# kfkq/DQMC

Hardware: AMD Instinct MI355X
Metric: MC sweeps/sec, 2D Hubbard N=256 Ltau=200 (higher is better)
Workload: dtype f64; 1 GPU; cfg3: 16x16 Hubbard U=8.0 beta=8.0 Ltau=200 n_stab=10 t=1 mu=-0.1; chains_per_gpu=1, n_chains_total=1, parallelism=independent chains, 1 gpu x 1 chain

## Files before the change

dqmc_amd/abi.py:

```python
from __future__ import annotations

import ctypes as C
import os
from typing import Optional, Tuple

import numpy as np

c_double_p = C.POINTER(C.c_double)
c_int64_p = C.POINTER(C.c_int64)
c_int32_p = C.POINTER(C.c_int32)
c_uint8_p = C.POINTER(C.c_uint8)
c_uint32_p = C.POINTER(C.c_uint32)
c_uint64_p = C.POINTER(C.c_uint64)


class Stats(C.Structure):
    _fields_ = [("acc_rate", C.c_double), ("max_err", C.c_double), ("sum_err", C.c_double),
                ("n_err", C.c_double), ("n_accepted", C.c_int64), ("n_proposed", C.c_int64)]

    @property
    def mean_err(self) -> float:
        return self.sum_err / self.n_err if self.n_err else 0.0


class DqmcError(RuntimeError):
    def __init__(self, code: int, msg: str):
        super().__init__(f"[{code}] {msg}")
        self.code = code


ABI_SYMBOLS = [
    "last_error", "backend", "device_count",
    "to_ldr", "ldr_mul_mat", "mat_mul_ldr", "ldr_mul_ldr", "inv_I_plus_ldr", "inv_I_plus_ldr_mul_ldr",
    "gemm", "rank1_update",
    "create", "create_batch", "n_chains", "destroy", "set_fields", "get_fields", "init", "get_G", "set_G", "get_logdet",
    "n_stack", "get_stack", "sweep_0_to_beta", "sweep_beta_to_0", "sync", "get_stats",
    "wrap_forward", "wrap_backward", "local_update_slice", "calculate_Bbar", "global_action", "set_checkerboard",
    "update_kernel_time", "set_profiling", "slice_path", "debug_snapshot", "debug_gt_check",
    "measure_equal_time", "measure_accumulate", "measure_fetch",
    "sweep_unequal_time", "get_G_tau", "half_warp", "measure_unequal_time", "measure_unequal_fetch",
    "comm_unique_id", "comm_create_rccl", "comm_create_callbacks", "comm_destroy", "comm_rank", "comm_world_size",
    "comm_transport", "comm_barrier", "comm_allreduce_sum", "comm_selftest", "partner_rank", "replica_exchange_round",
    "replica_exchange_batch",
    "rng_seed", "rng_state", "rng_draw", "rng_fill_time",
]

UNIQUE_ID_BYTES = 128
SENDRECV_FN = C.CFUNCTYPE(C.c_int, C.c_void_p, C.c_void_p, C.c_void_p, C.c_size_t, C.c_int, C.c_int)


class ExchangeResult(C.Structure):
    _fields_ = [("partner", C.c_int), ("decider", C.c_int), ("accepted", C.c_int), ("pad", C.c_int),
                ("S", C.c_double), ("S_prime", C.c_double), ("S_partner", C.c_double), ("S_prime_partner", C.c_double),
# ... 47 lines not shown
        if self.has_symbol("slice_path"):
            g("slice_path").argtypes = [C.c_void_p]
        if self.has_symbol("measure_equal_time"):
            g("measure_equal_time").argtypes = [C.c_void_p, C.c_int, C.c_int, c_double_p, c_double_p]
            g("measure_accumulate").argtypes = [C.c_void_p, C.c_int, C.c_int]
            g("measure_fetch").argtypes = [C.c_void_p, c_double_p, c_double_p, c_int64_p, C.c_int]
        if self.has_symbol("sweep_unequal_time"):
            g("sweep_unequal_time").argtypes = [C.c_void_p]
            g("get_G_tau").argtypes = [C.c_void_p, C.c_int, C.c_int, c_double_p]
            g("measure_unequal_time").argtypes = [C.c_void_p, C.c_int, C.c_int, C.c_int, c_double_p]
            g("measure_unequal_fetch").argtypes = [C.c_void_p, c_double_p, c_int64_p, C.c_int]
        if self.has_symbol("half_warp"):
            g("half_warp").argtypes = [C.c_void_p, c_double_p, c_double_p, C.c_int, C.c_int, c_double_p]
        if self.has_symbol("debug_snapshot"):
            g("debug_snapshot").argtypes = [C.c_void_p, c_double_p, C.c_void_p, C.c_void_p, C.c_void_p]
        if self.has_symbol("debug_gt_check"):
            g("debug_gt_check").argtypes = [C.c_void_p, C.c_int, c_double_p, c_int64_p]
        if self.has_symbol("replica_exchange_round"):
            g("comm_unique_id").argtypes = [C.c_void_p]
            g("comm_create_rccl").argtypes = [C.POINTER(C.c_void_p), C.c_void_p, C.c_int, C.c_int, C.c_int]
            g("comm_create_callbacks").argtypes = [C.POINTER(C.c_void_p), C.c_int, C.c_int, SENDRECV_FN, C.c_void_p]
            g("comm_destroy").argtypes = [C.c_void_p]; g("comm_destroy").restype = None
            g("comm_rank").argtypes = [C.c_void_p]; g("comm_world_size").argtypes = [C.c_void_p]
            g("comm_transport").argtypes = [C.c_void_p]; g("comm_transport").restype = C.c_char_p
            g("comm_barrier").argtypes = [C.c_void_p]; g("comm_selftest").argtypes = [C.c_void_p]
            g("comm_allreduce_sum").argtypes = [C.c_void_p, c_double_p, C.c_int]
            g("partner_rank").argtypes = [C.c_int, C.c_int, C.c_int]
            g("replica_exchange_round").argtypes = [C.c_void_p, C.c_void_p, C.c_int, C.c_double, C.POINTER(ExchangeResult)]
        if self.has_symbol("replica_exchange_batch"):
            g("replica_exchange_batch").argtypes = [C.c_void_p, C.c_void_p, C.c_int, c_double_p, C.POINTER(ExchangeResult)]
# ... 354 lines not shown
        out = np.empty(self.C * 3 * (self.nt + 1) * L1 * L2); cnt = np.zeros(1, dtype=np.int64)
        self._c("measure_unequal_fetch", _p(out), cnt.ctypes.data_as(c_int64_p), 1 if reset else 0)
        return self._ut_cube(out, L1, L2), int(cnt[0])

    def debug_snapshot(self):
        ns = self.n_stack()
        we = np.zeros(ns); acc = np.zeros(self.nt, np.int32); sw = np.zeros(80, np.uint32); ep = C.c_uint(0)
        self._c("debug_snapshot", _p(we), acc.ctypes.data, sw.ctypes.data, C.byref(ep))
        return dict(wrap_err=we, accepted=acc, sync_words=sw, slice_epoch=int(ep.value))

    def debug_gt_check(self, on: bool):
        err = np.zeros(self.C); cnt = np.zeros(1, dtype=np.int64)
        self._c("debug_gt_check", int(bool(on)), _p(err), cnt.ctypes.data_as(c_int64_p))
        return err, int(cnt[0])

    def slice_path(self) -> int:
        return int(self.lib._sym("slice_path")(self._h))

    def set_profiling(self, on: bool):
        self._c("set_profiling", int(bool(on)))

    def update_kernel_time(self):
        ms = C.c_double(0.0); nl = C.c_int64(0); na = C.c_int64(0)
        self._c("update_kernel_time", C.cast(C.byref(ms), c_double_p), C.cast(C.byref(nl), c_int64_p), C.cast(C.byref(na), c_int64_p))
        return ms.value, nl.value, na.value
```

dqmc_amd/csrc/common.h:

```cpp
#pragma once

#include <hip/hip_runtime.h>
#include <cstdint>
#include <memory>
#include <string>

struct dqmc_engine;

namespace dq {

constexpr int WAVE = 64;

void set_error(const std::string& msg);
const char* get_error();

#define DQ_HIP(call)                                                                    \
    do {                                                                                \
        hipError_t _e = (call);                                                         \
        if (_e != hipSuccess) {                                                         \
            ::dq::set_error(std::string(#call) + ": " + hipGetErrorString(_e));         \
            return -2;                                              \
        }                                                                               \
    } while (0)

// ... 88 lines not shown

int launch_tri_solve(CMat R, const int* perm, long perm_stride, Mat X, CVec dg, double* scratch, long scratch_stride, int n, int n_chains, hipStream_t s);

bool gj_fused_fits(int n);
bool gj_fused_default(int n);
int launch_gj_solve(Mat A, Mat B, Mat X, Mat SA, double* tinv, int* perm, long perm_stride, int* rowpos, int* rowpos_alt, long rowpos_stride,
                    double* logabsdet, int accumulate_logdet, int* info, int n, int n_chains, bool fused, hipStream_t s);

struct UpdateTables {
    double rb[4][3];
    double delta[4][3];
    double ev[4];
    double iev[4];
    double pad[32];
};
struct UpdateDesc {
    Mat G;
    int8_t* fields; long f_stride;
    double* expv; double* invexpv; long v_stride;
    const UpdateTables* tabs;
    const int32_t* perm; const uint8_t* kprop; const double* u; long rs_stride;
    double* Upanel; double* Wpanel; long panel_stride;
    double* Cpanel = nullptr;
    int* state; long state_stride;
    double* prep; long prep_stride;
    Mat GT{nullptr, 0};
    int gt_valid = 0;
    void* slice_sync = nullptr;
    unsigned slice_epoch = 0;
    int slice_absent_tile = -1;
    int slice_absent_l = -1;
    int slice_late_tile = -1, slice_late_us = 0;
    int* info = nullptr;
    int* acc_out; long acc_stride;
    int n, nt;
};
constexpr int UPDATE_KD = 32;

struct SliceSync {
    unsigned long long seq; unsigned int error; unsigned int solo_count; unsigned int pad[12];
    unsigned int arrive[496];
};
constexpr size_t SLICE_SYNC_BYTES = 2048;
static_assert(sizeof(SliceSync) == SLICE_SYNC_BYTES, "SliceSync layout");
constexpr unsigned SLICE_EPOCH_LIMIT = 1u << 24;
constexpr unsigned SLICE_SOLO_BIT = 1u << 30, SLICE_FINAL_BIT = 1u << 31;
__host__ __device__ inline unsigned slice_tag(unsigned epoch, unsigned window) { return (epoch << 8) | window; }
enum class SlicePath { PersistentWalk, PersistentSubmatrix, Solo, Pairs, PairsTailSolo };
int launch_update_slice(SlicePath path, const UpdateDesc& d, int l, int acc_slot, int n_chains, hipStream_t s);
int launch_update_slice_sm(const UpdateDesc& d, int l, int acc_slot, int n_chains, hipStream_t s);
// ... 32 lines not shown
```

dqmc_amd/csrc/engine.hip:

```cpp
#include "common.h"
#include "../../include/dqmc_hip.h"

#include <cmath>
#include <cstdlib>
#include <cstring>
#include <map>
#include <memory>
#include <mutex>
#include <vector>

namespace dq {

static thread_local std::string g_err;
void set_error(const std::string& msg) { g_err = msg; }
const char* get_error() { return g_err.c_str(); }

int init_device_kernels(int device) {
    static std::mutex mu; static bool done[64] = {};
    std::lock_guard<std::mutex> lk(mu);
    if (device < 0 || device >= 64) { set_error("device ordinal out of range"); return -1; }
    if (done[device]) return 0;
    DQ_HIP(hipSetDevice(device));
    DQ_TRY(update_init_device()); DQ_TRY(update_sm_init_device()); DQ_TRY(qr_init_device()); DQ_TRY(qr_colown_init_device());
    done[device] = true;
    return 0;
}

struct Switches { bool qr_panel; int qr_panel_fused, gj_fused; bool qr_streaming, walk_submatrix, lu_classic, slice_multikernel; };
static const Switches& switches() {
    static const Switches sw = [] {
        const char* panel = getenv("DQMC_QR_PANEL");
        const char* fused = getenv("DQMC_QR_PANEL_FUSED");
        const char* gj = getenv("DQMC_GJ_FUSED");
        return Switches{!(panel && atoi(panel) == 0), fused ? (atoi(fused) != 0 ? 1 : 0) : -1, gj ? (atoi(gj) != 0 ? 1 : 0) : -1, getenv("DQMC_QR_STREAMING") != nullptr, getenv("DQMC_WALK_SUBMATRIX") != nullptr,
                        getenv("DQMC_LU_CLASSIC") != nullptr, getenv("DQMC_SLICE_MULTIKERNEL") != nullptr};
    }();
    return sw;
}

constexpr int GJ_MAX_N = 1024, GJ_MAX_CHAINS = 8;
constexpr int TRI_MAX_N = 640;

static QrFamily pick_qr(int n, int chains, bool allow_panel) {
    const Switches& sw = switches();
    if (sw.qr_streaming) return QrFamily::Streaming;
    if (allow_panel && sw.qr_panel && n >= 64 && n <= 1024 && n % 16 == 0 && chains <= 8) return QrFamily::Panel;
    if (n <= 256) return QrFamily::ColumnOwner;
    return qrcp_coop_workgroups(n, chains) <= 200 ? QrFamily::Cooperative : QrFamily::Streaming;
}

// ... 229 lines not shown
    Ctx ctx;
    hipStream_t s = nullptr;

    DevPtr<double> expK, invexpK;
    bool cb = false; int cb_groups = 0;
    DevPtr<int> cb_partner;
    DevPtr<double> cb_par;
    DevPtr<int8_t> fields;
    DevPtr<double> expv, invexpv;
    DevPtr<UpdateTables> tabs; DevPtr<double> tab8;
    bool gt_valid = false;
    bool gt_check = false; long long gt_checks = 0; DevPtr<double> gt_err;
    DevPtr<double> G, Gtmp, GT;
    DevPtr<double> pg_eye, pg_ones;
    DevPtr<double> bb0, bb1;
    LdrStore stack;
    LdrStore spare;
    DevPtr<double> logdet;
    DevPtr<int32_t> rs_perm; DevPtr<uint8_t> rs_k; DevPtr<double> rs_u;
    PinnedPtr h_stage;
    bool rng_seeded = false; uint64_t rng_seed = 0; uint32_t rng_first_chain = 0, rng_counter = 0;
    hipEvent_t stage_free = nullptr;
    DevPtr<double> Upanel, Wpanel;
    DevPtr<double> Cpanel;
    struct InitBatch { DevPtr<double> bb, tau; LdrStore f; } ib;
    DevPtr<int> state;
    DevPtr<double> prep;
    DevPtr<double> meas_now, meas_sum;
    struct UnequalTime { DevPtr<double> G[3], tmp, err, meas_now, meas_sum; LdrStore bt; } ut;
    bool ut_valid = false; long long ut_meas_count = 0;
// ... 181 lines not shown
        stack_valid = true;
        gt_valid = false;
        return ctx.inv_I_plus_ldr(stack.at(0), mG(), logdet.get());
    }
    int wrap_forward(int l) {
        if (cb) {
            DQ_TRY(cb_apply(mG(), Mat{nullptr, 0}, ctx.T(0), false, false, CVec(), CVec(), CVec(), CVec(), C, 4));
            gt_valid = use_gt();
            return cb_apply(ctx.T(0), Mat{GT.get(), nn}, mG(), false, true, CVec(), CVec(), iev(l), ev(l), C, 4);
        }
        DQ_TRY(ctx.gemm(CMat(expK.get(), nn), mG(), ctx.T(0)));
        gt_valid = use_gt();
        return ctx.gemm(ctx.T(0), CMat(invexpK.get(), nn), mG(), ev(l), CVec(), iev(l), 0, 0, use_gt() ? Mat{GT.get(), nn} : Mat{nullptr, 0});
    }
    bool piggyback() const { return C == 1 && !cb && n <= 256 && pg_eye != nullptr; }
    int wrap_forward_piggy(int l, const double* Pprev, double* Pnext) {
        GemmDesc g; g.A = CMat(expK.get(), 0); g.B = CMat(G.get(), (long)(Pprev - G.get())); g.C = Mat{ctx.T(0).p, (long)(Pnext - ctx.T(0).p)};
        g.rs = CVec(pg_ones.get(), (long)((expv.get() + (long)(l - 1) * n) - pg_ones.get())); g.n = n;
        DQ_TRY(launch_gemm(g, 2, s));
        gt_valid = use_gt();
        return ctx.gemm(ctx.T(0), CMat(invexpK.get(), nn), mG(), ev(l), CVec(), iev(l), 0, 0, use_gt() ? Mat{GT.get(), nn} : Mat{nullptr, 0});
    }
    int wrap_backward_piggy(int l, const double* Pprev, double* Pnext) {
        DQ_TRY(ctx.gemm(CMat(invexpK.get(), nn), mG(), ctx.T(0), CVec(), iev(l)));
        gt_valid = use_gt();
        GemmDesc g; g.A = CMat(ctx.T(0).p, (long)(Pprev - ctx.T(0).p)); g.B = CMat(expK.get(), 0); g.C = Mat{G.get(), (long)(Pnext - G.get())};
        g.ks = CVec(expv.get() + (long)l * n, 0); g.n = n;
        if (use_gt()) g.CT = Mat{GT.get(), (long)(ctx.T(1).p - GT.get())};
        return launch_gemm(g, 2, s);
    }
// ... 2 lines not shown
            DQ_TRY(cb_apply(mG(), Mat{nullptr, 0}, ctx.T(0), true, true, iev(l), ev(l), CVec(), CVec(), C, 4));
            gt_valid = use_gt();
            return cb_apply(ctx.T(0), Mat{GT.get(), nn}, mG(), true, false, CVec(), CVec(), CVec(), CVec(), C, 4);
        }
        DQ_TRY(ctx.gemm(CMat(invexpK.get(), nn), mG(), ctx.T(0), CVec(), iev(l)));
        gt_valid = use_gt();
        return ctx.gemm(ctx.T(0), CMat(expK.get(), nn), mG(), CVec(), ev(l), CVec(), 0, 0, use_gt() ? Mat{GT.get(), nn} : Mat{nullptr, 0});
    }
    bool use_gt() const { return n <= 256 || slice_path == SlicePath::PersistentSubmatrix; }
    UpdateDesc udesc() const {
        UpdateDesc d; d.G = mG(); d.fields = fields.get(); d.f_stride = (long)nt * n; d.expv = expv.get(); d.invexpv = invexpv.get(); d.v_stride = (long)nt * n;
        d.tabs = tabs.get(); d.perm = rs_perm.get(); d.kprop = rs_k.get(); d.u = rs_u.get(); d.rs_stride = (long)nt * n; d.Upanel = Upanel.get(); d.Wpanel = Wpanel.get(); d.Cpanel = Cpanel.get();
        d.panel_stride = (long)UPDATE_KD * n; d.state = state.get(); d.state_stride = 4; d.prep = prep.get(); d.prep_stride = 4L * n; d.slice_sync = is_persistent(slice_path) ? slice_sync.get() : nullptr; d.slice_epoch = slice_epoch; d.slice_absent_tile = slice_absent_tile; d.slice_absent_l = slice_absent_l; d.slice_late_tile = slice_late_tile; d.slice_late_us = slice_late_us; d.GT = Mat{GT.get(), nn}; d.gt_valid = gt_valid ? 1 : 0; d.info = ctx.info(); d.acc_out = acc.get(); d.acc_stride = nt; d.n = n; d.nt = nt;
        return d;
    }
    int local_update(int l) {
        hipEvent_t e0 = nullptr, e1 = nullptr;
        if (profiling) {
            if (ev_used == ev_pairs.size()) { hipEvent_t a, b; DQ_HIP(hipEventCreate(&a)); DQ_HIP(hipEventCreate(&b)); ev_pairs.emplace_back(a, b); }
            e0 = ev_pairs[ev_used].first; e1 = ev_pairs[ev_used].second; ++ev_used;
            DQ_HIP(hipEventRecord(e0, s));
        }
        if (is_persistent(slice_path)) {
            if (++slice_epoch >= SLICE_EPOCH_LIMIT) { DQ_HIP(hipMemsetAsync(slice_sync.get(), 0, (size_t)C * SLICE_SYNC_BYTES, s)); slice_epoch = 1; }
        }
        DQ_TRY(launch_update_slice(slice_path, udesc(), l, l, C, s));
        if (profiling) DQ_HIP(hipEventRecord(e1, s));
        return 0;
    }
    int check_stream(const char* who, const int32_t* perm, const uint8_t* kprop, const double* u, size_t rows) {
        if (!perm || !kprop || !u) { set_error(std::string(who) + ": null random-stream pointer"); return DQMC_EINVAL; }
        seen.assign((size_t)n, 0);
        for (size_t row = 0; row < rows; ++row) {
            const int32_t* pr = perm + row * n; const uint8_t* kr = kprop + row * n; const unsigned char mark = (unsigned char)(1 + (row & 1));
            if ((row & 1) == 0) std::fill(seen.begin(), seen.end(), 0);
            for (int idx = 0; idx < n; ++idx) {
                const int32_t i = pr[idx];
                if (i < 0 || i >= n || seen[i] == mark || kr[idx] > 2) { set_error(std::string(who) + ": perm is not a permutation of the sites, or kprop > 2"); return DQMC_EINVAL; }
                seen[i] = mark;
            }
        }
// ... 17 lines not shown
    int fill_stream(uint32_t h) {
        return launch_rng_fill(rs_perm.get(), rs_k.get(), rs_u.get(), n, nt, rng_seed, rng_first_chain, h, C, s);
    }
    int stage_stream(const char* who, const int32_t* perm, const uint8_t* kprop, const double* u) {
        if (perm && kprop && u) return upload_stream(perm, kprop, u);
        if (perm || kprop || u) { set_error(std::string(who) + ": pass all three random-stream arrays or none"); return DQMC_EINVAL; }
        if (!rng_seeded) { set_error(std::string(who) + ": null random-stream pointer (the engine draws its own stream only after dqmc_rng_seed)"); return DQMC_EINVAL; }
        if (rng_counter == UINT32_MAX) { set_error(std::string(who) + ": the half-sweep counter of this seed is used up (2^32 - 1)"); return DQMC_ERANGE; }
        DQ_TRY(fill_stream(rng_counter));
        ++rng_counter;
        return 0;
    }
    int sweep_fwd() {
        int n_err = 0;
        DQ_HIP(hipMemsetAsync(err.get(), 0, sizeof(double) * C * n_stack, s));
        const bool pg = piggyback();
        double* Pcur = bb0.get(); double* Pnxt = bb1.get();
        for (int l = 0; l < nt; ++l) {
            const int is = stack_idx(l), loc = local_l(l);
            if (pg && loc >= 1) { DQ_TRY(wrap_forward_piggy(l, loc == 1 ? pg_eye.get() : Pcur, Pnxt)); std::swap(Pcur, Pnxt); }
            else DQ_TRY(wrap_forward(l));
            DQ_TRY(local_update(l));
            if (loc == loc_l_end[is]) {
                std::swap(G, Gtmp);
                Mat bb;
                if (pg) {
                    if (loc == 0) DQ_TRY(launch_scale_rows(CMat(expK.get(), nn), ev(l), Mat{Pnxt, nn}, n, C, s));
                    else DQ_TRY(ctx.gemm(CMat(expK.get(), nn), CMat(Pcur, nn), Mat{Pnxt, nn}, ev(l)));
                    std::swap(Pcur, Pnxt); bb = Mat{Pcur, nn};
                } else DQ_TRY(Bbar(is, &bb));
                if (is == 0) DQ_TRY(ctx.to_ldr(bb, stack.at(0)));
                else DQ_TRY(ctx.mat_mul_ldr(bb, stack.at(is - 1), stack.at(is)));
                gt_valid = false;
                if (l == nt - 1) DQ_TRY(ctx.inv_I_plus_ldr(stack.at(is), mG(), logdet.get()));
                else DQ_TRY(ctx.inv_I_plus_ldr_mul_ldr(stack.at(is), stack.at(is + 1), mG()));
                DQ_TRY(launch_max_abs_diff(CMat(Gtmp.get(), nn), mG(), err.get() + n_err, n_stack, n, C, s));
                ++n_err;
            }
        }
        return launch_fold_stats(dstats.get(), acc.get(), nt, nt, err.get(), n_stack, n_err, n, nt, C, s);
    }
    int sweep_bwd() {
        int n_err = 0;
        DQ_HIP(hipMemsetAsync(err.get(), 0, sizeof(double) * C * n_stack, s));
        const bool pg = piggyback();
        double* Pcur = bb0.get(); double* Pnxt = bb1.get();
        for (int l = nt - 1; l >= 0; --l) {
            DQ_TRY(local_update(l));
            const int is = stack_idx(l);
            if (pg) { DQ_TRY(wrap_backward_piggy(l, local_l(l) == loc_l_end[is] ? pg_eye.get() : Pcur, Pnxt)); std::swap(Pcur, Pnxt); }
            else DQ_TRY(wrap_backward(l));
            if (local_l(l) == 0) {
                std::swap(G, Gtmp);
                Mat bb;
                if (pg) bb = Mat{Pcur, nn}; else DQ_TRY(Bbar(is, &bb));
                if (is == n_stack - 1) DQ_TRY(ctx.to_ldr(bb, stack.at(is)));
                else DQ_TRY(ctx.ldr_mul_mat(stack.at(is + 1), bb, stack.at(is)));
                gt_valid = false;
                if (l == 0) DQ_TRY(ctx.inv_I_plus_ldr(stack.at(is), mG(), logdet.get()));
                else {
                    DQ_TRY(ctx.inv_I_plus_ldr_mul_ldr(stack.at(is - 1), stack.at(is), mG(), use_gt() ? Mat{GT.get(), nn} : Mat{nullptr, 0}));
                    gt_valid = use_gt();
                    if (gt_check && gt_valid) {
                        DQ_TRY(launch_transpose_scale(mG(), ctx.T(0), CVec(), n, C, s));
                        DQ_TRY(launch_max_abs_diff(CMat(GT.get(), nn), ctx.T(0), gt_err.get(), 1, n, C, s));
                        ++gt_checks;
// ... 502 lines not shown
    DQ_HIP(hipMemcpy(st.data(), e.dstats.get(), sizeof(DevStats) * e.C, hipMemcpyDeviceToHost));
    long long acc = 0; for (auto& x : st) acc += x.n_accepted;
    if (ms) *ms = e.upd_ms; if (n_launches) *n_launches = e.upd_launches; if (n_accepted) *n_accepted = acc - e.upd_accept_base;
    e.upd_ms = 0.0; e.upd_launches = 0; e.upd_accept_base = acc;
    return 0;
}
int dqmc_debug_snapshot(dqmc_engine* h, double* wrap_err, int* accepted, unsigned int* sync_words, unsigned int* slice_epoch) {
    ENGINE_CALL(h);
    DQ_HIP(hipStreamSynchronize(e.s));
    if (wrap_err) DQ_HIP(hipMemcpy(wrap_err, e.err.get(), sizeof(double) * e.n_stack, hipMemcpyDeviceToHost));
    if (accepted) DQ_HIP(hipMemcpy(accepted, e.acc.get(), sizeof(int) * e.nt, hipMemcpyDeviceToHost));
    if (sync_words) DQ_HIP(hipMemcpy(sync_words, e.slice_sync.get(), sizeof(unsigned int) * 80, hipMemcpyDeviceToHost));
    if (slice_epoch) *slice_epoch = e.slice_epoch;
    return 0;
}
int dqmc_debug_gt_check(dqmc_engine* h, int on, double* max_err, int64_t* n_checks) {
    ENGINE_CALL(h); DQ_TRY(e.sync_and_check());
    if (!e.gt_err) { DQ_TRY(dev_alloc(e.gt_err, e.C)); DQ_HIP(hipMemset(e.gt_err.get(), 0, sizeof(double) * e.C)); }
    if (max_err) DQ_HIP(hipMemcpy(max_err, e.gt_err.get(), sizeof(double) * e.C, hipMemcpyDeviceToHost));
    if (n_checks) *n_checks = e.gt_checks;
    DQ_HIP(hipMemset(e.gt_err.get(), 0, sizeof(double) * e.C));
    e.gt_checks = 0; e.gt_check = on != 0;
    return 0;
}
int dqmc_slice_path(dqmc_engine* h) {
    if (!h) return -1;
    Engine& e = h->e;
    if (!is_persistent(e.slice_path)) return 0;
    unsigned solo = 0;
    for (int c = 0; c < e.C && !solo; ++c) {
// ... 12 lines not shown
```

dqmc_amd/csrc/gemm.hip:

```cpp
#include "common.h"
#include <cstdlib>

namespace dq {

using d4 = __attribute__((ext_vector_type(4))) double;

template <bool TRANSA, bool GUARD>
__global__ __launch_bounds__(256) void gemm_kernel(GemmDesc g, int tiles_per_dim) {
    const int chain = blockIdx.y;
    const int n = g.n;
    const double* __restrict__ A = g.A.at(chain);
    const double* __restrict__ B = g.B.at(chain);
    double* __restrict__ C = g.C.at(chain);
    const double* __restrict__ ks = g.ks.p ? g.ks.at(chain) : nullptr;

    const int lane = threadIdx.x & 63;
    const int wave = threadIdx.x >> 6;
    const int bt_i = blockIdx.x % tiles_per_dim, bt_j = blockIdx.x / tiles_per_dim;
    const int i0 = bt_i * 32 + (wave & 1) * 16;
    const int j0 = bt_j * 32 + (wave >> 1) * 16;
    if (GUARD && (i0 >= n || j0 >= n)) return;

    const int r = lane & 15, kk = lane >> 4;
    const int ia = i0 + r;
// ... 27 lines not shown
            const int j = j0 + kk + 4 * reg;
            if (!GUARD || j < n) {
                double v = acc[reg] * rsv;
                if (g.cs.p) v *= g.cs.at(chain)[j];
                double* dst = C + ia + (long)n * j;
                if (g.accumulate) v += *dst;
                *dst = v;
            }
        }
    }
}

template <bool TRANSA, int KQ >
__global__ __launch_bounds__(256) void gemm_splitk_kernel(GemmDesc g, int tiles_per_dim) {
    __shared__ double part[4][4][64];
    const int chain = blockIdx.y;
    const int n = g.n;
    const double* __restrict__ A = g.A.at(chain);
    const double* __restrict__ B = g.B.at(chain);
    double* __restrict__ C = g.C.at(chain);
    const double* __restrict__ ks = g.ks.p ? g.ks.at(chain) : nullptr;
    const int lane = threadIdx.x & 63, wave = threadIdx.x >> 6;
    const int i0 = (blockIdx.x % tiles_per_dim) * 16, j0 = (blockIdx.x / tiles_per_dim) * 16;
    const int r = lane & 15, kk = lane >> 4;
    const int ia = min(i0 + r, n - 1), jb = min(j0 + r, n - 1);
    const bool ia_ok = i0 + r < n, jb_ok = j0 + r < n;
    const int kbeg = wave * KQ;
    constexpr int NB = KQ / 16;
    double av[NB][4], bv[NB][4];
#pragma unroll
    for (int b = 0; b < NB; ++b) {
#pragma unroll
        for (int s = 0; s < 4; ++s) {
            const int k = kbeg + 16 * b + 4 * kk + s;
            const int kc = min(k, n - 1);
            double a = TRANSA ? A[kc + (long)n * ia] : A[ia + (long)n * kc];
            double bb = B[kc + (long)n * jb];
            if (ks) a *= ks[kc];
            const bool ok = k < n;
            av[b][s] = (ok && ia_ok) ? a : 0.0;
            bv[b][s] = (ok && jb_ok) ? bb : 0.0;
        }
    }
    d4 acc = {0.0, 0.0, 0.0, 0.0};
#pragma unroll
    for (int b = 0; b < NB; ++b)
#pragma unroll
        for (int s = 0; s < 4; ++s) acc = __builtin_amdgcn_mfma_f64_16x16x4f64(bv[b][s], av[b][s], acc, 0, 0, 0);
#pragma unroll
    for (int reg = 0; reg < 4; ++reg) part[wave][reg][lane] = acc[reg];
    __syncthreads();
    const double v4 = part[0][wave][lane] + part[1][wave][lane] + part[2][wave][lane] + part[3][wave][lane];
    const int j = j0 + kk + 4 * wave;
    if (ia_ok && j < n) {
        double v = v4;
        if (g.rs.p) v *= g.rs.at(chain)[i0 + r];
        if (g.cs.p) v *= g.cs.at(chain)[j];
        double* dst = C + (i0 + r) + (long)n * j;
        if (g.accumulate) v += *dst;
        *dst = v;
        if (g.CT.p) g.CT.at(chain)[j + (long)n * (i0 + r)] = v;
    }
}

template <bool TRANSA>
__global__ __launch_bounds__(256) void gemm_tile64_kernel(GemmDesc g, int tiles_per_dim) {
    constexpr int LDT = 80;
    __shared__ double As[2][16][LDT];
    __shared__ double Bs[2][16][LDT];
    const int tiles2 = tiles_per_dim * tiles_per_dim;
    const int total = tiles2 * (int)gridDim.y;
    int lin = (int)blockIdx.x + tiles2 * (int)blockIdx.y;
    if ((total & 7) == 0) lin = (lin & 7) * (total >> 3) + (lin >> 3);
    const int chain = lin / tiles2, tile = lin % tiles2;
    const int n = g.n;
    const double* __restrict__ A = g.A.at(chain);
    const double* __restrict__ B = g.B.at(chain);
// ... 224 lines not shown
        else hipLaunchKernelGGL((gemm_tile64_kernel<false>), grid, block, 0, s, g, tiles);
        DQ_HIP(hipGetLastError());
        return 0;
    }
    if (n >= 384) {
        const int T = (n + 31) / 32, chunk = (T * T + 7) / 8;
        dim3 grid(8 * chunk, n_chains), block(256);
#define DQ_ST(TA, KSC) hipLaunchKernelGGL((gemm_stage32_kernel<TA, KSC, 32>), grid, block, 0, s, g, T, chunk)
        if (g.transA) { if (g.ks.p) DQ_ST(true, true); else DQ_ST(true, false); } else { if (g.ks.p) DQ_ST(false, true); else DQ_ST(false, false); }
#undef DQ_ST
        DQ_HIP(hipGetLastError());
        *ct_done = true;
        return 0;
    }
    if (n <= 640) {
        const int kq = ((n + 3) / 4 + 15) / 16 * 16;
        if (kq <= 16) launch_splitk<16>(g, n_chains, s);
        else if (kq <= 32) launch_splitk<32>(g, n_chains, s);
        else if (kq <= 48) launch_splitk<48>(g, n_chains, s);
        else if (kq <= 64) launch_splitk<64>(g, n_chains, s);
        else if (kq <= 96) launch_splitk<96>(g, n_chains, s);
        else if (kq <= 128) launch_splitk<128>(g, n_chains, s);
        else launch_splitk<160>(g, n_chains, s);
        DQ_HIP(hipGetLastError());
        *ct_done = true;
        return 0;
    }
    const int tiles = (n + 31) / 32;
    dim3 grid(tiles * tiles, n_chains), block(256);
    const bool guard = (n % 32) != 0;
    if (g.transA) {
// ... 12 lines not shown
```

dqmc_amd/csrc/update.hip:

```cpp
#include "common.h"
#include <cstdlib>
#include <mutex>
#include "wave.h"

namespace dq {

using d4 = __attribute__((ext_vector_type(4))) double;

__constant__ int c_proposal[4][3] = {{1, 2, 3}, {0, 2, 3}, {0, 1, 3}, {0, 1, 2}};

constexpr int SCAN_PF = 8;

__device__ __forceinline__ double ld_coh(const double* p) {
    return __longlong_as_double((long long)__hip_atomic_load(reinterpret_cast<const unsigned long long*>(p), __ATOMIC_RELAXED, __HIP_MEMORY_SCOPE_AGENT));
}
__device__ __forceinline__ void st_coh(double* p, double x) {
    __hip_atomic_store(reinterpret_cast<unsigned long long*>(p), (unsigned long long)__double_as_longlong(x), __ATOMIC_RELAXED, __HIP_MEMORY_SCOPE_AGENT);
}

__host__ __device__ inline size_t scan_lds_bytes(int n, int kd, bool regs) {
    const size_t base = (((size_t)16 * kd * n + (size_t)n * 32 + 256 + (size_t)n * 4 + (size_t)n) + 63) & ~(size_t)63;
    return base + (regs ? (size_t)n * 8 + 4 * (UPDATE_KD + 4) : 0);
}

// ... 526 lines not shown
#pragma unroll
        for (int reg = 0; reg < 4; ++reg) {
            const int bb = b0 + kk + 4 * reg, aa = a0 + kk + 4 * reg;
            if (a_ok && bb < n) G[a + (long)n * bb] = gv[q][reg] + acc[reg];
            if (b_ok && aa < n) GT[b + (long)n * aa] = gt[q][reg] + acc_t[reg];
        }
    }
}

__device__ __attribute__((noinline)) void solo_flush(double* G, double* GT, const double2* UW, int n, int k) {
    const int lane = threadIdx.x & 63, wave = threadIdx.x >> 6;
    const int tiles16 = (n + 15) / 16, n_st = tiles16 * tiles16;
    for (int st = wave; st < n_st; st += 4 * 4) flush_tiles_lds<4>(G, GT, UW, st, 4, n_st, tiles16, n, k, lane);
}

template <int NFIX, int KFIX>
__global__ __launch_bounds__(256) DQ_WALK_REGS void slice_kernel(UpdateDesc d, SliceSync* sync_p, int l, int acc_slot, int kd_arg, int tiles_arg, int* info) {
    extern __shared__ __attribute__((aligned(16))) unsigned char smem[];
    const int chain = blockIdx.y;
    const int n = NFIX ? NFIX : d.n;
    const int kd = KFIX ? KFIX : kd_arg;
    const int tiles_per_dim = NFIX ? (NFIX + 31) / 32 : tiles_arg;
    const int F = tiles_per_dim * tiles_per_dim;
    SliceSync* sy = sync_p + chain;
    double* __restrict__ G = d.G.at(chain);
    double* __restrict__ GT = d.GT.at(chain);
    double* __restrict__ Up = d.Upanel + (long)chain * d.panel_stride;
    double* __restrict__ Wp = d.Wpanel + (long)chain * d.panel_stride;
    const int t = threadIdx.x, lane = t & 63, wave = t >> 6;
    const unsigned epoch = d.slice_epoch;

    if (blockIdx.x > 0) {
        const int tile = blockIdx.x - 1;
        if (tile == d.slice_absent_tile && (d.slice_absent_l < 0 || d.slice_absent_l == l)) return;
        if (tile == d.slice_late_tile) {
            const unsigned long long t0 = wall_clock64();
            while (wall_clock64() - t0 < 100ull * (unsigned long long)d.slice_late_us) __builtin_amdgcn_s_sleep(64);
        }
        const int a0 = (tile % tiles_per_dim) * 32 + (wave & 1) * 16;
        const int b0 = (tile / tiles_per_dim) * 32 + (wave >> 1) * 16;
        if (t == 0) __hip_atomic_store(&sy->arrive[tile], slice_tag(epoch, 0), __ATOMIC_RELAXED, __HIP_MEMORY_SCOPE_AGENT);
        unsigned long long* bcast = reinterpret_cast<unsigned long long*>(smem);
        for (unsigned win = 1;; ++win) {
            if (wave == 0) {
                unsigned long long word = 0; unsigned spins = 0; bool give_up = false;
                for (;;) {
                    word = __hip_atomic_load(&sy->seq, __ATOMIC_RELAXED, __HIP_MEMORY_SCOPE_AGENT);
                    const unsigned tag = (unsigned)(word >> 32);
                    if (tag == slice_tag(epoch, win)) break;
                    if ((tag >> 8) == (slice_tag(epoch, 0) >> 8)) {
                        if ((unsigned)word & SLICE_SOLO_BIT) break;
                        if ((tag & 0xffu) > win) { give_up = true; break; }
                    }
                    if (++spins > SLICE_SPIN_LIMIT) { give_up = true; break; }
                    __builtin_amdgcn_s_sleep(1);
                }
// ... 173 lines not shown
int update_init_device() {
    DQ_HIP(hipFuncSetAttribute(reinterpret_cast<const void*>(scan_kernel<256>), hipFuncAttributeMaxDynamicSharedMemorySize, 160 * 1024));
    DQ_HIP(hipFuncSetAttribute(reinterpret_cast<const void*>(scan_kernel<1024>), hipFuncAttributeMaxDynamicSharedMemorySize, 160 * 1024));
    DQ_HIP(hipFuncSetAttribute(reinterpret_cast<const void*>(slice_kernel<0, 0>), hipFuncAttributeMaxDynamicSharedMemorySize, 160 * 1024));
    DQ_HIP(hipFuncSetAttribute(reinterpret_cast<const void*>(slice_kernel<256, UPDATE_KD>), hipFuncAttributeMaxDynamicSharedMemorySize, 160 * 1024));
    DQ_HIP(hipFuncSetAttribute(reinterpret_cast<const void*>(slice_solo_kernel), hipFuncAttributeMaxDynamicSharedMemorySize, 160 * 1024));
    return 0;
}

int launch_update_slice(SlicePath path, const UpdateDesc& d, int l, int acc_slot, int n_chains, hipStream_t s) {
    const int n = d.n;
    if (n > 1024) { set_error("local update kernel supports n_sites <= 1024"); return -1; }
    const int kd = pick_kd(n);
    const int threads = ((n + 63) / 64) * 64;
    const bool regs = threads <= 256;
    const size_t lds = scan_lds_bytes(n, kd, regs);
    const int tiles = (n + 31) / 32;
    if (!regs && path != SlicePath::Pairs && path != SlicePath::PersistentSubmatrix) { set_error("local update: the walk kernels of update.hip need n_sites <= 256"); return -1; }
    if (regs || path == SlicePath::PersistentSubmatrix) {
        if (!d.GT.p) { set_error("local update: transposed workspace missing"); return -1; }
        if (!d.gt_valid) { if (int rc = launch_transpose_scale(CMat(d.G.p, d.G.stride), d.GT, CVec(), n, n_chains, s)) return rc; }
    }
    switch (path) {
    case SlicePath::PersistentSubmatrix: return launch_update_slice_sm(d, l, acc_slot, n_chains, s);
    case SlicePath::PersistentWalk:
        if (!d.slice_sync) { set_error("persistent slice kernel: hand-off words missing"); return -1; }
        if (n == 256 && kd == UPDATE_KD)
            hipLaunchKernelGGL((slice_kernel<256, UPDATE_KD>), dim3(1 + tiles * tiles, n_chains), dim3(256), lds, s, d, reinterpret_cast<SliceSync*>(d.slice_sync), l, acc_slot, kd,
                               tiles, d.info);
        else
            hipLaunchKernelGGL((slice_kernel<0, 0>), dim3(1 + tiles * tiles, n_chains), dim3(256), lds, s, d, reinterpret_cast<SliceSync*>(d.slice_sync), l, acc_slot, kd,
                               tiles, d.info);
        DQ_HIP(hipGetLastError());
        return 0;
    case SlicePath::Solo:
        hipLaunchKernelGGL(slice_solo_kernel, dim3(1, n_chains), dim3(256), lds, s, d, l, acc_slot, kd, 0);
        DQ_HIP(hipGetLastError());
        return 0;
    case SlicePath::Pairs: case SlicePath::PairsTailSolo: break;
    }
    int windows = (n + kd - 1) / kd;
// ... 49 lines not shown
```

include/dqmc_hip.h:

```cpp
#ifndef DQMC_HIP_H
#define DQMC_HIP_H

#include <stddef.h>
#include <stdint.h>

#ifdef __cplusplus
extern "C" {
#endif

#define DQMC_OK         0
#define DQMC_EINVAL    -1
#define DQMC_ENODEVICE -2
#define DQMC_ENUMERIC  -3
#define DQMC_ERANGE    -4
#define DQMC_ENOMEM    -5

typedef struct dqmc_engine dqmc_engine;

typedef struct dqmc_stats {
    double  acc_rate;
    double  max_err;
    double  sum_err;
    double  n_err;
    int64_t n_accepted;
// ... 112 lines not shown
    double S_prime;
    double S_partner;
    double S_prime_partner;
    double deltaS;
} dqmc_exchange_result;

int dqmc_replica_exchange_round(dqmc_engine* e, dqmc_comm* comm, int exchange_attempt, double u,
                                dqmc_exchange_result* result);

int dqmc_replica_exchange_batch(dqmc_engine* e, dqmc_comm* comm, int exchange_attempt, const double* u,
                                dqmc_exchange_result* result);

int dqmc_update_kernel_time(dqmc_engine* e, double* ms, int64_t* n_launches, int64_t* n_accepted);
int dqmc_slice_path(dqmc_engine* e);
int dqmc_debug_snapshot(dqmc_engine* e, double* wrap_err, int* accepted, unsigned int* sync_words, unsigned int* slice_epoch);
int dqmc_debug_gt_check(dqmc_engine* e, int on, double* max_err, int64_t* n_checks);
int dqmc_set_profiling(dqmc_engine* e, int on);

#ifdef __cplusplus
}
#endif
#endif
```

Before: 13.18 sweeps/s.

## Fuse the piggyback B-bar product GEMM into the persistent slice-update kernel

The running product of slice B matrices (the piggyback GEMM) is no longer launched as its own split-K kernel. It now rides inside the persistent walk slice kernel: the tile blocks compute GEMM tiles before they enter the hand-off loop. The split-K tile body moves into a shared header so both kernels can use it. This removes one kernel launch per time slice and overlaps the GEMM with the update kernel. In exchange it adds work and LDS to the update blocks before they sync, and the backward sweep has to defer the product by one slice.

```diff
diff --git a/dqmc_amd/abi.py b/dqmc_amd/abi.py
--- a/dqmc_amd/abi.py
+++ b/dqmc_amd/abi.py
@@ -36,7 +36,7 @@
     "create", "create_batch", "n_chains", "destroy", "set_fields", "get_fields", "init", "get_G", "set_G", "get_logdet",
     "n_stack", "get_stack", "sweep_0_to_beta", "sweep_beta_to_0", "sync", "get_stats",
     "wrap_forward", "wrap_backward", "local_update_slice", "calculate_Bbar", "global_action", "set_checkerboard",
-    "update_kernel_time", "set_profiling", "slice_path", "debug_snapshot", "debug_gt_check",
+    "update_kernel_time", "set_profiling", "slice_path", "debug_snapshot", "bbar_rider_launches", "debug_gt_check",
     "measure_equal_time", "measure_accumulate", "measure_fetch",
     "sweep_unequal_time", "get_G_tau", "half_warp", "measure_unequal_time", "measure_unequal_fetch",
     "comm_unique_id", "comm_create_rccl", "comm_create_callbacks", "comm_destroy", "comm_rank", "comm_world_size",
@@ -114,6 +114,8 @@
             g("half_warp").argtypes = [C.c_void_p, c_double_p, c_double_p, C.c_int, C.c_int, c_double_p]
         if self.has_symbol("debug_snapshot"):
             g("debug_snapshot").argtypes = [C.c_void_p, c_double_p, C.c_void_p, C.c_void_p, C.c_void_p]
+        if self.has_symbol("bbar_rider_launches"):
+            g("bbar_rider_launches").argtypes = [C.c_void_p, c_int64_p]
         if self.has_symbol("debug_gt_check"):
             g("debug_gt_check").argtypes = [C.c_void_p, C.c_int, c_double_p, c_int64_p]
         if self.has_symbol("replica_exchange_round"):
@@ -498,6 +500,9 @@
         self._c("debug_gt_check", int(bool(on)), _p(err), cnt.ctypes.data_as(c_int64_p))
         return err, int(cnt[0])
 
+    def bbar_rider_launches(self) -> int:
+        n = C.c_int64(0); self._c("bbar_rider_launches", C.byref(n)); return int(n.value)
+
     def slice_path(self) -> int:
         return int(self.lib._sym("slice_path")(self._h))
 
diff --git a/dqmc_amd/csrc/common.h b/dqmc_amd/csrc/common.h
--- a/dqmc_amd/csrc/common.h
+++ b/dqmc_amd/csrc/common.h
@@ -126,6 +126,10 @@
     double iev[4];
     double pad[32];
 };
+struct SliceRider {
+    const double* A = nullptr; const double* B = nullptr; double* C = nullptr; const double* rs = nullptr; const double* ks = nullptr;
+    __host__ __device__ GemmDesc gemm(int n) const { GemmDesc g; g.A = CMat(A, 0); g.B = CMat(B, 0); g.C = Mat{C, 0}; g.rs = CVec(rs, 0); g.ks = CVec(ks, 0); g.n = n; return g; }
+};
 struct UpdateDesc {
     Mat G;
     int8_t* fields; long f_stride;
@@ -146,6 +150,7 @@
     int* info = nullptr;
     int* acc_out; long acc_stride;
     int n, nt;
+    SliceRider rider;
 };
 constexpr int UPDATE_KD = 32;
 
diff --git a/dqmc_amd/csrc/engine.hip b/dqmc_amd/csrc/engine.hip
--- a/dqmc_amd/csrc/engine.hip
+++ b/dqmc_amd/csrc/engine.hip
@@ -26,14 +26,15 @@
     return 0;
 }
 
-struct Switches { bool qr_panel; int qr_panel_fused, gj_fused; bool qr_streaming, walk_submatrix, lu_classic, slice_multikernel; };
+struct Switches { bool qr_panel; int qr_panel_fused, gj_fused; bool qr_streaming, walk_submatrix, lu_classic, slice_multikernel, bbar_rider; };
 static const Switches& switches() {
     static const Switches sw = [] {
         const char* panel = getenv("DQMC_QR_PANEL");
         const char* fused = getenv("DQMC_QR_PANEL_FUSED");
         const char* gj = getenv("DQMC_GJ_FUSED");
+        const char* rider = getenv("DQMC_BBAR_RIDER");
         return Switches{!(panel && atoi(panel) == 0), fused ? (atoi(fused) != 0 ? 1 : 0) : -1, gj ? (atoi(gj) != 0 ? 1 : 0) : -1, getenv("DQMC_QR_STREAMING") != nullptr, getenv("DQMC_WALK_SUBMATRIX") != nullptr,
-                        getenv("DQMC_LU_CLASSIC") != nullptr, getenv("DQMC_SLICE_MULTIKERNEL") != nullptr};
+                        getenv("DQMC_LU_CLASSIC") != nullptr, getenv("DQMC_SLICE_MULTIKERNEL") != nullptr, !(rider && atoi(rider) == 0)};
     }();
     return sw;
 }
@@ -293,6 +294,7 @@
     DevPtr<double> G, Gtmp, GT;
     DevPtr<double> pg_eye, pg_ones;
     DevPtr<double> bb0, bb1;
+    long long rider_launches = 0;
     LdrStore stack;
     LdrStore spare;
     DevPtr<double> logdet;
@@ -504,6 +506,15 @@
         return ctx.gemm(ctx.T(0), CMat(invexpK.get(), nn), mG(), ev(l), CVec(), iev(l), 0, 0, use_gt() ? Mat{GT.get(), nn} : Mat{nullptr, 0});
     }
     bool piggyback() const { return C == 1 && !cb && n <= 256 && pg_eye != nullptr; }
+    bool bbar_rides() const { return piggyback() && slice_path == SlicePath::PersistentWalk && switches().bbar_rider; }
+    SliceRider rider_forward(int l, const double* Pprev, double* Pnext) const {
+        SliceRider r; r.A = expK.get(); r.B = Pprev; r.C = Pnext; r.rs = expv.get() + (long)(l - 1) * n;
+        return r;
+    }
+    SliceRider rider_backward(int l, const double* Pprev, double* Pnext) const {
+        SliceRider r; r.A = Pprev; r.B = expK.get(); r.C = Pnext; r.ks = expv.get() + (long)l * n;
+        return r;
+    }
     int wrap_forward_piggy(int l, const double* Pprev, double* Pnext) {
         GemmDesc g; g.A = CMat(expK.get(), 0); g.B = CMat(G.get(), (long)(Pprev - G.get())); g.C = Mat{ctx.T(0).p, (long)(Pnext - ctx.T(0).p)};
         g.rs = CVec(pg_ones.get(), (long)((expv.get() + (long)(l - 1) * n) - pg_ones.get())); g.n = n;
@@ -536,7 +547,7 @@
         d.panel_stride = (long)UPDATE_KD * n; d.state = state.get(); d.state_stride = 4; d.prep = prep.get(); d.prep_stride = 4L * n; d.slice_sync = is_persistent(slice_path) ? slice_sync.get() : nullptr; d.slice_epoch = slice_epoch; d.slice_absent_tile = slice_absent_tile; d.slice_absent_l = slice_absent_l; d.slice_late_tile = slice_late_tile; d.slice_late_us = slice_late_us; d.GT = Mat{GT.get(), nn}; d.gt_valid = gt_valid ? 1 : 0; d.info = ctx.info(); d.acc_out = acc.get(); d.acc_stride = nt; d.n = n; d.nt = nt;
         return d;
     }
-    int local_update(int l) {
+    int local_update(int l, const SliceRider* rider = nullptr) {
         hipEvent_t e0 = nullptr, e1 = nullptr;
         if (profiling) {
             if (ev_used == ev_pairs.size()) { hipEvent_t a, b; DQ_HIP(hipEventCreate(&a)); DQ_HIP(hipEventCreate(&b)); ev_pairs.emplace_back(a, b); }
@@ -546,7 +557,10 @@
         if (is_persistent(slice_path)) {
             if (++slice_epoch >= SLICE_EPOCH_LIMIT) { DQ_HIP(hipMemsetAsync(slice_sync.get(), 0, (size_t)C * SLICE_SYNC_BYTES, s)); slice_epoch = 1; }
         }
-        DQ_TRY(launch_update_slice(slice_path, udesc(), l, l, C, s));
+        UpdateDesc d = udesc();
+        if (rider) d.rider = *rider;
+        DQ_TRY(launch_update_slice(slice_path, d, l, l, C, s));
+        if (rider) ++rider_launches;
         if (profiling) DQ_HIP(hipEventRecord(e1, s));
         return 0;
     }
@@ -594,13 +608,16 @@
     int sweep_fwd() {
         int n_err = 0;
         DQ_HIP(hipMemsetAsync(err.get(), 0, sizeof(double) * C * n_stack, s));
-        const bool pg = piggyback();
+        const bool pg = piggyback(), ride = bbar_rides();
         double* Pcur = bb0.get(); double* Pnxt = bb1.get();
         for (int l = 0; l < nt; ++l) {
             const int is = stack_idx(l), loc = local_l(l);
-            if (pg && loc >= 1) { DQ_TRY(wrap_forward_piggy(l, loc == 1 ? pg_eye.get() : Pcur, Pnxt)); std::swap(Pcur, Pnxt); }
-            else DQ_TRY(wrap_forward(l));
-            DQ_TRY(local_update(l));
+            if (pg && loc >= 1) {
+                const double* Pprev = loc == 1 ? pg_eye.get() : Pcur;
+                if (ride) { const SliceRider r = rider_forward(l, Pprev, Pnxt); DQ_TRY(wrap_forward(l)); DQ_TRY(local_update(l, &r)); }
+                else { DQ_TRY(wrap_forward_piggy(l, Pprev, Pnxt)); DQ_TRY(local_update(l)); }
+                std::swap(Pcur, Pnxt);
+            } else { DQ_TRY(wrap_forward(l)); DQ_TRY(local_update(l)); }
             if (loc == loc_l_end[is]) {
                 std::swap(G, Gtmp);
                 Mat bb;
@@ -623,13 +640,18 @@
     int sweep_bwd() {
         int n_err = 0;
         DQ_HIP(hipMemsetAsync(err.get(), 0, sizeof(double) * C * n_stack, s));
-        const bool pg = piggyback();
+        const bool pg = piggyback(), ride = bbar_rides();
         double* Pcur = bb0.get(); double* Pnxt = bb1.get();
+        SliceRider pending; bool have_pending = false;
         for (int l = nt - 1; l >= 0; --l) {
-            DQ_TRY(local_update(l));
+            DQ_TRY(local_update(l, have_pending ? &pending : nullptr));
+            if (have_pending) { std::swap(Pcur, Pnxt); have_pending = false; }
             const int is = stack_idx(l);
-            if (pg) { DQ_TRY(wrap_backward_piggy(l, local_l(l) == loc_l_end[is] ? pg_eye.get() : Pcur, Pnxt)); std::swap(Pcur, Pnxt); }
-            else DQ_TRY(wrap_backward(l));
+            if (pg) {
+                const double* Pprev = local_l(l) == loc_l_end[is] ? pg_eye.get() : Pcur;
+                if (ride && local_l(l) != 0) { DQ_TRY(wrap_backward(l)); pending = rider_backward(l, Pprev, Pnxt); have_pending = true; }
+                else { DQ_TRY(wrap_backward_piggy(l, Pprev, Pnxt)); std::swap(Pcur, Pnxt); }
+            } else DQ_TRY(wrap_backward(l));
             if (local_l(l) == 0) {
                 std::swap(G, Gtmp);
                 Mat bb;
@@ -1162,6 +1184,11 @@
     if (slice_epoch) *slice_epoch = e.slice_epoch;
     return 0;
 }
+int dqmc_bbar_rider_launches(dqmc_engine* h, int64_t* n_launches) {
+    ENGINE_CALL(h);
+    if (n_launches) *n_launches = e.rider_launches;
+    return 0;
+}
 int dqmc_debug_gt_check(dqmc_engine* h, int on, double* max_err, int64_t* n_checks) {
     ENGINE_CALL(h); DQ_TRY(e.sync_and_check());
     if (!e.gt_err) { DQ_TRY(dev_alloc(e.gt_err, e.C)); DQ_HIP(hipMemset(e.gt_err.get(), 0, sizeof(double) * e.C)); }
diff --git a/dqmc_amd/csrc/gemm.hip b/dqmc_amd/csrc/gemm.hip
--- a/dqmc_amd/csrc/gemm.hip
+++ b/dqmc_amd/csrc/gemm.hip
@@ -1,4 +1,5 @@
 #include "common.h"
+#include "gemm_tile.h"
 #include <cstdlib>
 
 namespace dq {
@@ -65,53 +66,7 @@
 template <bool TRANSA, int KQ >
 __global__ __launch_bounds__(256) void gemm_splitk_kernel(GemmDesc g, int tiles_per_dim) {
     __shared__ double part[4][4][64];
-    const int chain = blockIdx.y;
-    const int n = g.n;
-    const double* __restrict__ A = g.A.at(chain);
-    const double* __restrict__ B = g.B.at(chain);
-    double* __restrict__ C = g.C.at(chain);
-    const double* __restrict__ ks = g.ks.p ? g.ks.at(chain) : nullptr;
-    const int lane = threadIdx.x & 63, wave = threadIdx.x >> 6;
-    const int i0 = (blockIdx.x % tiles_per_dim) * 16, j0 = (blockIdx.x / tiles_per_dim) * 16;
-    const int r = lane & 15, kk = lane >> 4;
-    const int ia = min(i0 + r, n - 1), jb = min(j0 + r, n - 1);
-    const bool ia_ok = i0 + r < n, jb_ok = j0 + r < n;
-    const int kbeg = wave * KQ;
-    constexpr int NB = KQ / 16;
-    double av[NB][4], bv[NB][4];
-#pragma unroll
-    for (int b = 0; b < NB; ++b) {
-#pragma unroll
-        for (int s = 0; s < 4; ++s) {
-            const int k = kbeg + 16 * b + 4 * kk + s;
-            const int kc = min(k, n - 1);
-            double a = TRANSA ? A[kc + (long)n * ia] : A[ia + (long)n * kc];
-            double bb = B[kc + (long)n * jb];
-            if (ks) a *= ks[kc];
-            const bool ok = k < n;
-            av[b][s] = (ok && ia_ok) ? a : 0.0;
-            bv[b][s] = (ok && jb_ok) ? bb : 0.0;
-        }
-    }
-    d4 acc = {0.0, 0.0, 0.0, 0.0};
-#pragma unroll
-    for (int b = 0; b < NB; ++b)
-#pragma unroll
-        for (int s = 0; s < 4; ++s) acc = __builtin_amdgcn_mfma_f64_16x16x4f64(bv[b][s], av[b][s], acc, 0, 0, 0);
-#pragma unroll
-    for (int reg = 0; reg < 4; ++reg) part[wave][reg][lane] = acc[reg];
-    __syncthreads();
-    const double v4 = part[0][wave][lane] + part[1][wave][lane] + part[2][wave][lane] + part[3][wave][lane];
-    const int j = j0 + kk + 4 * wave;
-    if (ia_ok && j < n) {
-        double v = v4;
-        if (g.rs.p) v *= g.rs.at(chain)[i0 + r];
-        if (g.cs.p) v *= g.cs.at(chain)[j];
-        double* dst = C + (i0 + r) + (long)n * j;
-        if (g.accumulate) v += *dst;
-        *dst = v;
-        if (g.CT.p) g.CT.at(chain)[j + (long)n * (i0 + r)] = v;
-    }
+    gemm_splitk_tile<TRANSA, KQ>(g, blockIdx.y, (blockIdx.x % tiles_per_dim) * 16, (blockIdx.x / tiles_per_dim) * 16, part);
 }
 
 template <bool TRANSA>
@@ -366,7 +321,7 @@
         return 0;
     }
     if (n <= 640) {
-        const int kq = ((n + 3) / 4 + 15) / 16 * 16;
+        const int kq = gemm_splitk_kq(n);
         if (kq <= 16) launch_splitk<16>(g, n_chains, s);
         else if (kq <= 32) launch_splitk<32>(g, n_chains, s);
         else if (kq <= 48) launch_splitk<48>(g, n_chains, s);
diff --git a/dqmc_amd/csrc/gemm_tile.h b/dqmc_amd/csrc/gemm_tile.h
--- /dev/null
+++ b/dqmc_amd/csrc/gemm_tile.h
@@ -0,0 +1,62 @@
+#pragma once
+
+#include "common.h"
+
+namespace dq {
+
+__host__ __device__ inline int gemm_splitk_kq(int n) { return ((n + 3) / 4 + 15) / 16 * 16; }
+
+template <bool TRANSA, int KQ>
+__device__ __forceinline__ void gemm_splitk_tile(const GemmDesc& g, int chain, int i0, int j0, double (*part)[4][64], int kq = KQ) {
+    using d4 = __attribute__((ext_vector_type(4))) double;
+    const int n = g.n;
+    const double* __restrict__ A = g.A.at(chain);
+    const double* __restrict__ B = g.B.at(chain);
+    double* __restrict__ C = g.C.at(chain);
+    const double* __restrict__ ks = g.ks.p ? g.ks.at(chain) : nullptr;
+    const int lane = threadIdx.x & 63, wave = threadIdx.x >> 6;
+    const int r = lane & 15, kk = lane >> 4;
+    const int ia = min(i0 + r, n - 1), jb = min(j0 + r, n - 1);
+    const bool ia_ok = i0 + r < n, jb_ok = j0 + r < n;
+    const int kbeg = wave * kq;
+    constexpr int NB = KQ / 16;
+    double av[NB][4], bv[NB][4];
+#pragma unroll
+    for (int b = 0; b < NB; ++b) {
+        if (16 * b >= kq) break;
+#pragma unroll
+        for (int s = 0; s < 4; ++s) {
+            const int k = kbeg + 16 * b + 4 * kk + s;
+            const int kc = min(k, n - 1);
+            double a = TRANSA ? A[kc + (long)n * ia] : A[ia + (long)n * kc];
+            double bb = B[kc + (long)n * jb];
+            if (ks) a *= ks[kc];
+            const bool ok = k < n;
+            av[b][s] = (ok && ia_ok) ? a : 0.0;
+            bv[b][s] = (ok && jb_ok) ? bb : 0.0;
+        }
+    }
+    d4 acc = {0.0, 0.0, 0.0, 0.0};
+#pragma unroll
+    for (int b = 0; b < NB; ++b) {
+        if (16 * b >= kq) break;
+#pragma unroll
+        for (int s = 0; s < 4; ++s) acc = __builtin_amdgcn_mfma_f64_16x16x4f64(bv[b][s], av[b][s], acc, 0, 0, 0);
+    }
+#pragma unroll
+    for (int reg = 0; reg < 4; ++reg) part[wave][reg][lane] = acc[reg];
+    __syncthreads();
+    const double v4 = part[0][wave][lane] + part[1][wave][lane] + part[2][wave][lane] + part[3][wave][lane];
+    const int j = j0 + kk + 4 * wave;
+    if (ia_ok && j < n) {
+        double v = v4;
+        if (g.rs.p) v *= g.rs.at(chain)[i0 + r];
+        if (g.cs.p) v *= g.cs.at(chain)[j];
+        double* dst = C + (i0 + r) + (long)n * j;
+        if (g.accumulate) v += *dst;
+        *dst = v;
+        if (g.CT.p) g.CT.at(chain)[j + (long)n * (i0 + r)] = v;
+    }
+}
+
+}
diff --git a/dqmc_amd/csrc/update.hip b/dqmc_amd/csrc/update.hip
--- a/dqmc_amd/csrc/update.hip
+++ b/dqmc_amd/csrc/update.hip
@@ -2,6 +2,7 @@
 #include <cstdlib>
 #include <mutex>
 #include "wave.h"
+#include "gemm_tile.h"
 
 namespace dq {
 
@@ -564,6 +565,23 @@
     for (int st = wave; st < n_st; st += 4 * 4) flush_tiles_lds<4>(G, GT, UW, st, 4, n_st, tiles16, n, k, lane);
 }
 
+constexpr size_t SLICE_RIDER_LDS_OFF = 16;
+constexpr size_t SLICE_RIDER_LDS = SLICE_RIDER_LDS_OFF + sizeof(double) * 4 * 4 * 64;
+template <int NFIX>
+__device__ __forceinline__ void slice_rider(const SliceRider& rd, int n, int f, int F, unsigned char* smem) {
+    if (__builtin_expect(!rd.C, 1)) return;
+    const GemmDesc g = rd.gemm(n);
+    const int chain = 0;
+    double (*part)[4][64] = reinterpret_cast<double (*)[4][64]>(smem + SLICE_RIDER_LDS_OFF);
+    const int T = (n + 15) / 16;
+    const int kq = NFIX ? gemm_splitk_kq(NFIX) : gemm_splitk_kq(n);
+    for (int tile = f; tile < T * T; tile += F) {
+        const int i0 = (tile % T) * 16, j0 = (tile / T) * 16;
+        gemm_splitk_tile<false, 64>(g, chain, i0, j0, part, kq);
+        __syncthreads();
+    }
+}
+
 template <int NFIX, int KFIX>
 __global__ __launch_bounds__(256) DQ_WALK_REGS void slice_kernel(UpdateDesc d, SliceSync* sync_p, int l, int acc_slot, int kd_arg, int tiles_arg, int* info) {
     extern __shared__ __attribute__((aligned(16))) unsigned char smem[];
@@ -582,14 +600,16 @@
 
     if (blockIdx.x > 0) {
         const int tile = blockIdx.x - 1;
-        if (tile == d.slice_absent_tile && (d.slice_absent_l < 0 || d.slice_absent_l == l)) return;
-        if (tile == d.slice_late_tile) {
+        const bool absent = tile == d.slice_absent_tile && (d.slice_absent_l < 0 || d.slice_absent_l == l);
+        if (!absent && tile == d.slice_late_tile) {
             const unsigned long long t0 = wall_clock64();
             while (wall_clock64() - t0 < 100ull * (unsigned long long)d.slice_late_us) __builtin_amdgcn_s_sleep(64);
         }
         const int a0 = (tile % tiles_per_dim) * 32 + (wave & 1) * 16;
         const int b0 = (tile / tiles_per_dim) * 32 + (wave >> 1) * 16;
-        if (t == 0) __hip_atomic_store(&sy->arrive[tile], slice_tag(epoch, 0), __ATOMIC_RELAXED, __HIP_MEMORY_SCOPE_AGENT);
+        if (!absent && t == 0) __hip_atomic_store(&sy->arrive[tile], slice_tag(epoch, 0), __ATOMIC_RELAXED, __HIP_MEMORY_SCOPE_AGENT);
+        slice_rider<NFIX>(d.rider, n, tile, F, smem);
+        if (absent) return;
         unsigned long long* bcast = reinterpret_cast<unsigned long long*>(smem);
         for (unsigned win = 1;; ++win) {
             if (wave == 0) {
@@ -793,7 +813,7 @@
     const int kd = pick_kd(n);
     const int threads = ((n + 63) / 64) * 64;
     const bool regs = threads <= 256;
-    const size_t lds = scan_lds_bytes(n, kd, regs);
+    size_t lds = scan_lds_bytes(n, kd, regs);
     const int tiles = (n + 31) / 32;
     if (!regs && path != SlicePath::Pairs && path != SlicePath::PersistentSubmatrix) { set_error("local update: the walk kernels of update.hip need n_sites <= 256"); return -1; }
     if (regs || path == SlicePath::PersistentSubmatrix) {
@@ -804,6 +824,15 @@
     case SlicePath::PersistentSubmatrix: return launch_update_slice_sm(d, l, acc_slot, n_chains, s);
     case SlicePath::PersistentWalk:
         if (!d.slice_sync) { set_error("persistent slice kernel: hand-off words missing"); return -1; }
+        if (d.rider.C) {
+            if (n_chains != 1 || !d.rider.A || !d.rider.B) { set_error("persistent slice kernel: malformed rider product"); return -1; }
+            if (gemm_splitk_kq(n) > 64) { set_error("persistent slice kernel: the rider's split-K instance covers n <= 256"); return -1; }
+            const double* rows[2] = {d.expv + (long)l * n, d.invexpv + (long)l * n};
+            for (const double* v : {d.rider.rs, d.rider.ks})
+                for (const double* row : rows)
+                    if (v && row && v + n > row && v < row + n) { set_error("persistent slice kernel: the rider reads the e^V row of the slice this launch walks"); return -1; }
+            if (lds < SLICE_RIDER_LDS) lds = SLICE_RIDER_LDS;
+        }
         if (n == 256 && kd == UPDATE_KD)
             hipLaunchKernelGGL((slice_kernel<256, UPDATE_KD>), dim3(1 + tiles * tiles, n_chains), dim3(256), lds, s, d, reinterpret_cast<SliceSync*>(d.slice_sync), l, acc_slot, kd,
                                tiles, d.info);
diff --git a/include/dqmc_hip.h b/include/dqmc_hip.h
--- a/include/dqmc_hip.h
+++ b/include/dqmc_hip.h
@@ -150,6 +150,7 @@
 int dqmc_update_kernel_time(dqmc_engine* e, double* ms, int64_t* n_launches, int64_t* n_accepted);
 int dqmc_slice_path(dqmc_engine* e);
 int dqmc_debug_snapshot(dqmc_engine* e, double* wrap_err, int* accepted, unsigned int* sync_words, unsigned int* slice_epoch);
+int dqmc_bbar_rider_launches(dqmc_engine* e, int64_t* n_launches);
 int dqmc_debug_gt_check(dqmc_engine* e, int on, double* max_err, int64_t* n_checks);
 int dqmc_set_profiling(dqmc_engine* e, int on);
 
```

After: 13.35 sweeps/s (median of 6 runs). 1.3% higher.
